# acids-ircam/RAVE

Hardware: NVIDIA H100
Metric: audio-seconds/s (v2 train step fwd+bwd, 48 kHz) (higher is better)
Workload: dtype bf16

## Files before the change

include/rave_b200.h:

```cpp
#ifndef RAVE_B200_H
#define RAVE_B200_H

#include <stddef.h>
#include <stdint.h>

#ifdef __cplusplus
extern "C" {
#endif

#define RAVE_ACT_NONE 0
#define RAVE_ACT_LEAKY 1
#define RAVE_ACT_SNAKE 2

#define RAVE_PREC_FP32 0
#define RAVE_PREC_BF16 1
#define RAVE_PREC_TF32 2

int rave_b200_version(void);
const char *rave_b200_last_error(void);
unsigned long long rave_b200_launch_count(void);

int rave_pqmf_analysis_fwd(const float *x, const float *taps, float *y, int B, int T, int Lout,
                           int ntaps, int pad_l, int flip_sign, void *stream);
int rave_pqmf_synthesis_fwd(const float *x, const float *w, float *out, int B, int L, int K,
// ... 19 lines not shown
                          int Lq, int K, int stride, int dil, int pad_l, long os_a, long os_c,
                          int act_p, int act_q, float slope, const float *alpha, void *workspace,
                          void *stream);

int rave_weight_norm_fwd(const float *v, const float *g, float *w, float *norm_out, int C0, int R,
                         void *stream);
int rave_weight_norm_bwd(const float *dw, const float *v, const float *g, const float *norm,
                         float *dv, float *dg, int C0, int R, void *stream);

int rave_act_fwd(const float *x, float *y, int B, int C, int L, int act, float slope,
                 const float *alpha, void *stream);
int rave_act_bwd(const float *dy, const float *x, float *dx, float *dalpha, int B, int C, int L,
                 int act, float slope, const float *alpha, void *stream);
int rave_am_tanh_fwd(const float *x, float *y, int B, int C, int L, void *stream);
int rave_am_tanh_bwd(const float *dy, const float *x, float *dx, int B, int C, int L, void *stream);
int rave_reparam_fwd(const float *z, const float *eps, float *zs, float *kl_sum, int B, int C, int L, void *stream);
int rave_mmd_fwd(const float *z, const float *prior, float *means, float *mmd, int B, int D, int L, void *stream);
int rave_mmd_bwd(const float *z, const float *prior, const float *g, float *dz, int B, int D, int L, void *stream);
int rave_sphere_norm_fwd(const float *z, float *out, float *norm, int B, int C, int L, void *stream);
int  rave_latent_moments(const float *z, int B, int C, int L, int D, double *state, double *work, void *stream);
long rave_latent_moments_workspace_bytes(int B, int L, int D);
int rave_sphere_norm_bwd(const float *g, const float *out, const float *norm, float *dz, int B, int C, int L,
                         void *stream);

int rave_conv1d_tc_supported(int Cin, int Cout, int K, int stride, int dil);
int rave_dilated_unit_tc_supported(int C, int L);
int rave_dilated_unit_tc_fwd(const void *xa_bf16, const void *w3t_bf16, const void *w1t_bf16, void *a1_out,
                             float *out_f32, void *out_act, int B, int C, int L, int pitch, int dil, int pad_l,
                             float slope_in, float slope_mid, int act_out, float slope_out, void *stream);
int rave_conv1d_tc_plan(int B, int Cin, int Cout, int Lout, int K);
int rave_conv1d_tc_pp_stages(int B, int Cin, int Cout, int Lout, int K, int fm, int res_bf16);
int rave_conv1d_tc_pp_fwd_stages(int B, int Cin, int Cout, int Lout, int K);
int rave_conv1d_tc_wide_stages(int B, int Cin, int Cout, int Lout, int K);
int rave_conv1d_tc_fwd(const void *xa_bf16, const void *wt_bf16, const float *bias, const float *res,
                       const void *res_bf16, const void *dact_src_bf16, const void *res_act_bf16, float res_slope,
                       float *out_f32, void *out_act_bf16,
                       int B, int Cin, int Lin, int in_pitch, int Cout, int Lout,
                       int K, int stride, int dil, int pad_l, int act, float slope, int out_rows,
                       int out_row_stride, int out_row_offset, const float *fm_d, int fm_bh, void *stream);
int rave_conv1d_tc_fwd_x3(const void *xa_bf16, const void *wt_bf16, const float *bias, const float *res,
                          const void *res_act, float res_slope, float *out_f32, void *out_act, int B, int Cin, int Lin,
                          int in_pitch, int Cout, int Lout, int K, int stride, int dil, int pad_l, int act, float slope,
                          int out_rows, int out_row_stride, int out_row_offset, int act_cs, void *stream);
int rave_conv1d_tc_wgrad_splits(int B, int Cm, int Lp, int Cn, int K);
int rave_conv1d_tc_wgrad_plan(int B, int Cm, int Lp, int Cn, int K);
int rave_time_stack_cl(const float *x, void *out_bf16, int B, int C, int T, int F, int Fp, int Cp, int kt, int pt,
                       void *stream);
int rave_time_stack_cl_bwd(const void *g_bf16, float *gx, int B, int C, int T, int F, int Fp, int Cp, int kt, int pt,
                           void *stream);
int rave_time_stack_nhwc(const float *x, void *out_bf16, int B, int C, int T, int F, long sb, long st, int Fp, int Cp, int kt,
                         int pt, void *stream);
int rave_time_stack_nhwc_bwd(const void *g_bf16, float *gx, int B, int C, int T, int F, int Fp, int Cp, int kt, int pt,
                             void *stream);
int rave_time_stack_nhwc_dil(const float *x, void *out_bf16, int B, int C, int T, int F, long sb, long st, int Fp, int Cp,
                             int kt, int pt, int dil, void *stream);
int rave_time_stack_nhwc_dil_bwd(const void *g_bf16, float *gx, int B, int C, int T, int F, int Fp, int Cp, int kt, int pt,
                                 int dil, void *stream);
int rave_l1_stats_f32(const float *t, const float *v, float *stats, long n, void *stream);
int rave_l1_grad_f32(const float *t, const float *v, const float *d, float *gt, float *gv, long n, void *stream);
int rave_leaky_fm_fwd(const float *x, float *a, float *stats, long H, float slope, void *stream);
int rave_leaky_fm_bwd(const float *a, const float *g, const float *d, float *gx, long H, float slope, void *stream);
int rave_leaky_fm_stack_fwd(const float *x, float *a, float *stats, void *xs_bf16, long Rh, int T, int F, int C, int Fp,
                            float slope, void *stream);
int rave_leaky_fm_stack_bwd(const float *a, const void *gxs_bf16, const float *ga, const float *d, float *gx, long Rh, int T,
                            int F, int C, int Fp, float slope, void *stream);
int rave_leaky_fm_stack_dil_fwd(const float *x, float *a, float *stats, void *xs_bf16, long Rh, int T, int F, int C, int Fp,
// ... 147 lines not shown
```

rave_b200/_lib.py:

```python
import ctypes
import os
from ctypes import c_float, c_int, c_long, c_longlong, c_size_t, c_ulonglong, c_void_p, c_char_p

_HERE = os.path.dirname(os.path.abspath(__file__))
LIB_PATH = os.path.join(_HERE, "csrc", "librave_b200.so")

_P, _I, _F, _L = c_void_p, c_int, c_float, c_long

SIGNATURES = {
    "rave_b200_version": (c_int, []),
    "rave_b200_last_error": (c_char_p, []),
    "rave_b200_launch_count": (c_ulonglong, []),
    "rave_pqmf_analysis_fwd": (c_int, [_P, _P, _P, _I, _I, _I, _I, _I, _I, _P]),
    "rave_pqmf_synthesis_fwd": (c_int, [_P, _P, _P, _I, _I, _I, _I, _F, _I, _P]),
    "rave_pqmf_analysis_fast": (c_int, [_P, _P, _P, _P, _I, _I, _I, _I, _I, _P]),
    "rave_pqmf_synthesis_fast": (c_int, [_P, _P, _P, _P, _I, _I, _I, _F, _I, _P]),
    "rave_conv1d_gather_f32": (c_int, [_P, _P, _P, _P, _P, _I, _I, _I, _I, _I, _I, _I, _I, _I, _L, _L,
                                       _I, _F, _P, _I, _F, _P, _P, _P]),
    "rave_conv1d_scatter_f32": (c_int, [_P, _P, _P, _P, _P, _I, _I, _I, _I, _I, _I, _I, _I, _I, _L, _L,
                                        _I, _F, _P, _I, _F, _P, _P, _P]),
    "rave_conv1d_wgrad_workspace_bytes": (c_size_t, [_I, _I, _I, _I, _I]),
    "rave_conv1d_wgrad_f32": (c_int, [_P, _P, _P, _I, _I, _I, _I, _I, _I, _I, _I, _I, _L, _L, _I, _I,
                                      _F, _P, _P, _P]),
    "rave_weight_norm_fwd": (c_int, [_P, _P, _P, _P, _I, _I, _P]),
    "rave_weight_norm_bwd": (c_int, [_P, _P, _P, _P, _P, _P, _I, _I, _P]),
    "rave_act_fwd": (c_int, [_P, _P, _I, _I, _I, _I, _F, _P, _P]),
    "rave_act_bwd": (c_int, [_P, _P, _P, _P, _I, _I, _I, _I, _F, _P, _P]),
    "rave_am_tanh_fwd": (c_int, [_P, _P, _I, _I, _I, _P]),
    "rave_am_tanh_bwd": (c_int, [_P, _P, _P, _I, _I, _I, _P]),
    "rave_reparam_fwd": (c_int, [_P, _P, _P, _P, _I, _I, _I, _P]),
    "rave_mmd_fwd": (c_int, [_P, _P, _P, _P, _I, _I, _I, _P]),
    "rave_mmd_bwd": (c_int, [_P, _P, _P, _P, _I, _I, _I, _P]),
    "rave_sphere_norm_fwd": (c_int, [_P, _P, _P, _I, _I, _I, _P]),
    "rave_sphere_norm_bwd": (c_int, [_P, _P, _P, _P, _I, _I, _I, _P]),
    "rave_latent_moments": (c_int, [_P, _I, _I, _I, _I, _P, _P, _P]),
    "rave_latent_moments_workspace_bytes": (c_long, [_I, _I, _I]),
    "rave_conv1d_tc_supported": (c_int, [_I, _I, _I, _I, _I]),
    "rave_dilated_unit_tc_supported": (c_int, [_I, _I]),
    "rave_dilated_unit_tc_fwd": (c_int, [_P, _P, _P, _P, _P, _P, _I, _I, _I, _I, _I, _I, _F, _F, _I, _F, _P]),
    "rave_conv1d_tc_plan": (c_int, [_I, _I, _I, _I, _I]),
    "rave_conv1d_tc_pp_stages": (c_int, [_I, _I, _I, _I, _I, _I, _I]),
    "rave_conv1d_tc_pp_fwd_stages": (c_int, [_I, _I, _I, _I, _I]),
    "rave_conv1d_tc_wide_stages": (c_int, [_I, _I, _I, _I, _I]),
    "rave_conv1d_tc_fwd": (c_int, [_P, _P, _P, _P, _P, _P, _P, _F, _P, _P, _I, _I, _I, _I, _I, _I, _I, _I, _I, _I, _I,
                                   _F, _I, _I, _I, _P, _I, _P]),
    "rave_conv1d_tc_fwd_x3": (c_int, [_P, _P, _P, _P, _P, _F, _P, _P, _I, _I, _I, _I, _I, _I, _I, _I, _I, _I, _I, _F, _I,
                                      _I, _I, _I, _P]),
    "rave_weight_prep_tc_multi_x3": (c_int, [_I, _P, _P]),
    "rave_ncl_to_cl_x3": (c_int, [_P, _P, _I, _I, _I, _P]),
    "rave_conv1d_tc_wgrad": (c_int, [_P, _P, _P, _P, _I, _I, _I, _I, _I, _I, _I, _I, _I, _I, _I, _P]),
    "rave_tapmajor_to_weight_f32": (c_int, [_P, _P, _I, _I, _I, _I, _I, _P]),
    "rave_conv1d_tc_wgrad_splits": (c_int, [_I, _I, _I, _I, _I]),
    "rave_conv1d_tc_wgrad_plan": (c_int, [_I, _I, _I, _I, _I]),
    "rave_time_stack_cl": (c_int, [_P, _P, _I, _I, _I, _I, _I, _I, _I, _I, _P]),
    "rave_time_stack_cl_bwd": (c_int, [_P, _P, _I, _I, _I, _I, _I, _I, _I, _I, _P]),
    "rave_time_stack_nhwc": (c_int, [_P, _P, _I, _I, _I, _I, ctypes.c_long, ctypes.c_long, _I, _I, _I, _I, _P]),
    "rave_time_stack_nhwc_bwd": (c_int, [_P, _P, _I, _I, _I, _I, _I, _I, _I, _I, _P]),
    "rave_time_stack_nhwc_dil": (c_int, [_P, _P, _I, _I, _I, _I, ctypes.c_long, ctypes.c_long, _I, _I, _I, _I, _I, _P]),
    "rave_time_stack_nhwc_dil_bwd": (c_int, [_P, _P, _I, _I, _I, _I, _I, _I, _I, _I, _I, _P]),
    "rave_l1_stats_f32": (c_int, [_P, _P, _P, ctypes.c_long, _P]),
    "rave_leaky_fm_fwd": (c_int, [_P, _P, _P, ctypes.c_long, ctypes.c_float, _P]),
    "rave_leaky_fm_bwd": (c_int, [_P, _P, _P, _P, ctypes.c_long, ctypes.c_float, _P]),
    "rave_leaky_fm_stack_fwd": (c_int, [_P, _P, _P, _P, ctypes.c_long, _I, _I, _I, _I, ctypes.c_float, _P]),
    "rave_leaky_fm_stack_bwd": (c_int, [_P, _P, _P, _P, _P, ctypes.c_long, _I, _I, _I, _I, ctypes.c_float, _P]),
    "rave_leaky_fm_stack_dil_fwd": (c_int, [_P, _P, _P, _P, ctypes.c_long, _I, _I, _I, _I, _I, ctypes.c_float, _P]),
    "rave_leaky_fm_stack_dil_bwd": (c_int, [_P, _P, _P, _P, _P, ctypes.c_long, _I, _I, _I, _I, _I, ctypes.c_float, _P]),
    "rave_l1_grad_f32": (c_int, [_P, _P, _P, _P, _P, ctypes.c_long, _P]),
    "rave_snake_cl_fwd": (c_int, [_P, _P, _P, ctypes.c_long, _I, _P]),
    "rave_snake_cl_bwd": (c_int, [_P, _P, _P, _P, _P, _P, ctypes.c_long, _I, _P]),
    "rave_adain_cl_stats": (c_int, [_P, _I, _I, _I, _I, _P, _P, _P, _P, _P, _P, _P, _P, _I, _P, _P, _P]),
    "rave_adain_snake_cl_fwd": (c_int, [_P, _P, _P, _P, _P, _I, _I, _I, _I, _P]),
    "rave_weight_prep_tc": (c_int, [_P, _P, _P, _P, _P, _I, _P, _P, _I, _I, _I, _I, _I, _I, _P]),
    "rave_weight_norm_bwd_tapmajor": (c_int, [_P, _P, _P, _P, _P, _P, _I, _I, _I, _I, _I, _I, _P]),
    "rave_conv1d_c1_fwd": (c_int, [_P, _P, _P, _P, _P, _I, _I, _I, _I, _I, _I, _I, _I, _I, _I, _F, _P]),
    "rave_conv1d_c1_wgrad_splits": (c_int, [_I, _I]),
    "rave_conv1d_c1_wgrad": (c_int, [_P, _P, _P, _I, _I, _I, _I, _I, _I, _I, _I, _I, _I, _P]),
# ... 133 lines not shown
```

rave_b200/csrc/conv_tc.cu:

```cuda
#include <string.h>

#include <type_traits>

#include "common.cuh"
#include "tc_common.cuh"

namespace rave {
namespace tc {

constexpr int BLOCK_M = 128;
constexpr int NUM_THREADS = 288;
constexpr int SMEM_MAX = 227 * 1024;

struct TcParams {
  int B, Cin, Lin, Cout, Lout, K, stride, dil, pad_l;
  int BL, BB;
  int n_lt, n_bg, n_nt;
  int num_kb;
  int act;
  float slope;
  const float *bias;
  const float *res;
  const __nv_bfloat16 *res_bf16;
  const __nv_bfloat16 *dact_src;
// ... 391 lines not shown
      const bool valid = (b < p.B) && (l < p.Lout);
      const size_t orow = (size_t)b * p.out_rows + (size_t)l * p.out_row_stride + p.out_row_offset;

      const int buf = p.nacc == 2 ? (it & 1) : 0;
      const uint32_t use = p.nacc == 2 ? (it >> 1) : it;
      if (stg) {
        if (issuer) bulk_wait_read<0>();
        named_bar_sync(1, 128);
      }
      mbar_wait(&tfull_bar[buf], use & 1);
      const uint32_t taddr = (uint32_t)(128 * buf + quad * 32) << 16;
      tc_epilogue<BLOCK_N, X3, BOXC>(p, taddr, n0, valid, orow, p.fm_d ? (b < p.fm_bh ? 1 : -1) : 0, stg, row);
      __syncwarp();
      if (lane == 0) mbar_arrive(&tempty_bar[buf]);
      if (stg) {
        fence_proxy_async();
        named_bar_sync(1, 128);
        if (issuer) {
#pragma unroll
          for (int c = 0; c < BLOCK_N; c += BOXC)
            tma_store_3d(&tmap_o, stg + (c / BOXC) * (BLOCK_M * L::OUT_SPAN), n0 + c, t.l0, t.b0);
          bulk_commit();
        }
      }
    }
    if (stg && issuer) bulk_wait_all();
  }
}

constexpr int PP_THREADS = 384;

enum PpEpi : int { PP_FM = 1, PP_RS = 2, PP_FWD = 4, PP_BIAS = 8, PP_LEAKY = 16 };

template <int BLOCK_N, int BOXC, bool FM, bool RS>
__device__ __forceinline__ void pp_epilogue(float (*d)[BLOCK_N / 2], uint8_t *slot, const TcParams &p, int w, int lane,
                                            int b0) {
  constexpr int TILE_BYTES = BLOCK_M * BLOCK_N * 2;
  uint8_t *part = slot + TILE_BYTES;
  uint8_t *skip = slot + (FM ? 2 : 1) * TILE_BYTES;
  constexpr int SPAN = BOXC * 2, JB = BOXC / 8;
  const float d0 = FM ? __ldg(p.fm_d) : 0.f, d1 = FM ? __ldg(p.fm_d + 1) : 0.f;
  const uint32_t base = stg_offset<BOXC>(16 * w + (lane >> 2), 0) + 4 * (lane & 3);
#pragma unroll
  for (int h = 0; h < 2; ++h) {
#pragma unroll
    for (int r = 0; r < 2; ++r) {
      const int row = 64 * h + 16 * w + (lane >> 2) + 8 * r;
      const float d1r = (FM && b0 + row / p.BL < p.fm_bh) ? d1 : 0.f;
#pragma unroll
      for (int j = 0; j < BLOCK_N / 8; ++j) {
        const uint32_t off = (base ^ (uint32_t)((j % JB) << 4)) + (j / JB) * (BLOCK_M * SPAN) + (64 * h + 8 * r) * SPAN;
        float v0 = d[h][4 * j + 2 * r], v1 = d[h][4 * j + 2 * r + 1];
        const uint32_t dm = *reinterpret_cast<const uint32_t *>(slot + off);
        lrelu_mask(v0, v1, dm, p.slope);
        if (FM) fm_grad(v0, v1, dm, *reinterpret_cast<const uint32_t *>(part + off), d0, d1r);
        if (RS) add_bf16_pair(v0, v1, *reinterpret_cast<const uint32_t *>(skip + off));
        __nv_bfloat162 o = __floats2bfloat162_rn(v0, v1);
        *reinterpret_cast<uint32_t *>(slot + off) = *reinterpret_cast<uint32_t *>(&o);
      }
    }
  }
}

template <int BLOCK_N, int BOXC, bool BIAS, bool LEAKY, int NH = 2>
__device__ __forceinline__ void pp_fwd_epilogue(float (*d)[BLOCK_N / 2], uint8_t *slot, const TcParams &p, int w,
                                                int lane, int n0, int h0 = 0) {
  constexpr int SPAN = BOXC * 2, JB = BOXC / 8;
  const uint32_t base = stg_offset<BOXC>(16 * w + (lane >> 2), 0) + 4 * (lane & 3);
  const uint32_t sslot = smem_u32(slot);
  const float2 *bias = reinterpret_cast<const float2 *>(p.bias + n0 + 2 * (lane & 3));
#pragma unroll
  for (int j = 0; j < BLOCK_N / 8; ++j) {
    const float2 bb = BIAS ? __ldg(bias + 4 * j) : make_float2(0.f, 0.f);
    const uint32_t col = (base ^ (uint32_t)((j % JB) << 4)) + (j / JB) * (BLOCK_M * SPAN);
#pragma unroll
    for (int h = 0; h < NH; ++h) {
#pragma unroll
      for (int r = 0; r < 2; ++r) {
        float v0 = d[h][4 * j + 2 * r], v1 = d[h][4 * j + 2 * r + 1];
        if (BIAS) {
          v0 += bb.x;
          v1 += bb.y;
        }
        if (LEAKY) {
// ... 128 lines not shown
      if (issuer) {
#pragma unroll
        for (int cb = 0; cb < BLOCK_N / BOXC; ++cb)
          tma_store_3d(tmap_o, slot + cb * BOX_BYTES, t.n0 + cb * BOXC, t.l0, t.b0);
        bulk_commit();
        bulk_wait_read<0>();
        mbar_arrive(&oempty_bar[c]);
      }
    }
    if (issuer) bulk_wait_all();
  }
}

template <int BLOCK_N, int BLOCK_K, bool FM, bool RS>
__global__ void __launch_bounds__(PP_THREADS, 1)
conv_tc_pp_kernel(const __grid_constant__ CUtensorMap tmap_a, const __grid_constant__ CUtensorMap tmap_b,
                  const __grid_constant__ CUtensorMap tmap_m, const __grid_constant__ CUtensorMap tmap_p,
                  const __grid_constant__ CUtensorMap tmap_r, const __grid_constant__ CUtensorMap tmap_o,
                  const TcParams p) {
  conv_tc_pp_body<BLOCK_N, BLOCK_K, (FM ? PP_FM : 0) | (RS ? PP_RS : 0)>(&tmap_a, &tmap_b, &tmap_m, &tmap_p, &tmap_r,
                                                                         &tmap_o, p);
}

template <int BLOCK_N, int BLOCK_K, bool BIAS, bool LEAKY>
__global__ void __launch_bounds__(PP_THREADS, 1)
conv_tc_pp_fwd_kernel(const __grid_constant__ CUtensorMap tmap_a, const __grid_constant__ CUtensorMap tmap_b,
                      const __grid_constant__ CUtensorMap tmap_o, const TcParams p) {
  conv_tc_pp_body<BLOCK_N, BLOCK_K, PP_FWD | (BIAS ? PP_BIAS : 0) | (LEAKY ? PP_LEAKY : 0)>(
      &tmap_a, &tmap_b, nullptr, nullptr, nullptr, &tmap_o, p);
}

constexpr int WIDE_N = 192;

template <int BLOCK_K, bool BIAS, bool LEAKY>
__global__ void __launch_bounds__(PP_THREADS, 1)
conv_tc_wide_kernel(const __grid_constant__ CUtensorMap tmap_a, const __grid_constant__ CUtensorMap tmap_b,
                    const __grid_constant__ CUtensorMap tmap_o, const TcParams p) {
  constexpr int BLOCK_N = WIDE_N;
  using L = SmemLayout<BLOCK_N, BLOCK_K, false>;
  constexpr int BOXC = L::OUT_BOXC;
  constexpr int BOX_BYTES = BLOCK_M * L::OUT_SPAN;
  const int STAGES = p.stages;

  extern __shared__ uint8_t smem_raw[];
  uint8_t *smem = reinterpret_cast<uint8_t *>((reinterpret_cast<uintptr_t>(smem_raw) + 1023) & ~uintptr_t(1023));
  uint64_t *full_bar = reinterpret_cast<uint64_t *>(smem + p.bar_off);
  uint64_t *empty_bar = full_bar + STAGES;
  uint64_t *oempty_bar = empty_bar + STAGES;

  const int wg = threadIdx.x >> 7;
  const int warp = threadIdx.x >> 5;
  const int lane = threadIdx.x & 31;
  const int num_tiles = p.n_lt * p.n_bg * p.n_nt;
  const int kblocks = p.K * p.num_kb;

  if (threadIdx.x == 0) {
    tma_prefetch_desc(&tmap_a);
    tma_prefetch_desc(&tmap_b);
    tma_prefetch_desc(&tmap_o);
    for (int s = 0; s < STAGES; ++s) {
      mbar_init(&full_bar[s], 1);
      mbar_init(&empty_bar[s], 8);
    }
    mbar_init(oempty_bar, 1);
    fence_barrier_init();
  }
  __syncthreads();
  griddep_launch_dependents();
  griddep_wait();

  Ring ring{full_bar, empty_bar, STAGES, 0, 0};
  if (wg == 0) {
    warpgroup_reg_dealloc<56>();
    if (warp != 0) return;
    for (int tile = blockIdx.x; tile < num_tiles; tile += gridDim.x) {
      const TileCoord t = tile_coord<BLOCK_N>(tile, p);
      for (int k = 0; k < p.K; ++k) {
        const TapOrigin o = tap_origin(k, p.dil, p.pad_l, p.stride);
        for (int kb = 0; kb < p.num_kb; ++kb)
          produce_kblock<BLOCK_N, BLOCK_K, false>(smem, ring, &tmap_a, &tmap_b, p, t, o, k, kb);
      }
    }
  } else {
    warpgroup_reg_alloc<224>();
    const int h = wg - 1;
    const int w = warp & 3;
    const bool issuer = threadIdx.x == 128;
    const uint32_t smem_base = smem_u32(smem);
    uint8_t *slot = smem + p.ops_off;
    float d[1][BLOCK_N / 2];
    int u = 0;
    for (int tile = blockIdx.x; tile < num_tiles; tile += gridDim.x, ++u) {
      const int prev = mma_mainloop<BLOCK_N, BLOCK_K, false, 1>(d, smem_base, ring, kblocks, lane, h);
      mma_drain<BLOCK_N, 1>(d, ring, prev, lane);
      const TileCoord t = tile_coord<BLOCK_N>(tile, p);
      if (issuer && u > 0) {
        bulk_wait_read<0>();
        mbar_arrive(oempty_bar);
      }
      mbar_wait(oempty_bar, (u & 1) ^ 1);
      pp_fwd_epilogue<BLOCK_N, BOXC, BIAS, LEAKY, 1>(d, slot, p, w, lane, t.n0, h);
      fence_proxy_async();
      named_bar_sync(1, 256);
      if (issuer) {
#pragma unroll
        for (int cb = 0; cb < BLOCK_N / BOXC; ++cb)
          tma_store_3d(&tmap_o, slot + cb * BOX_BYTES, t.n0 + cb * BOXC, t.l0, t.b0);
        bulk_commit();
      }
    }
    if (issuer) bulk_wait_all();
  }
}

static CUtensorMapSwizzle swizzle_enum(int bytes) {
  return bytes == 128 ? CU_TENSOR_MAP_SWIZZLE_128B : bytes == 64 ? CU_TENSOR_MAP_SWIZZLE_64B
                                                                 : CU_TENSOR_MAP_SWIZZLE_32B;
}

static int pick_block_k(int Cin) {
  if (Cin % 64 == 0) return 64;
  if (Cin % 32 == 0) return 32;
  if (Cin % 16 == 0) return 16;
  return 0;
}

static int pick_block_n(int Cout, long m_tiles) {
  const int cands[] = {128, 96, 64, 48, 32, 16};
  constexpr int NC = sizeof(cands) / sizeof(cands[0]);
  int best = 0;
  for (int c : cands) {
    if (Cout % c) continue;
    if (!best) best = c;
    if (m_tiles * (Cout / c) >= 132) return c;
  }
  for (int i = NC - 1; i >= 0; --i)
    if (Cout % cands[i] == 0 && cands[i] >= 32) return cands[i];
  return best;
}

struct TcGeometry {
  int BK, BL, BB, n_lt, n_bg, BN, n_nt, num_kb;
};
static TcGeometry tc_geometry(int B, int Cin, int Cout, int Lout) {
  TcGeometry g;
// ... 40 lines not shown
  const cuuint64_t dims[3] = {(cuuint64_t)p.Cout, (cuuint64_t)p.Lout, (cuuint64_t)p.B};
  const cuuint64_t strides[2] = {(cuuint64_t)p.Cout * 2 * p.out_row_stride, (cuuint64_t)p.Cout * 2 * p.out_rows};
  const cuuint32_t box[3] = {(cuuint32_t)L::OUT_BOXC, (cuuint32_t)p.BL, (cuuint32_t)box_b};
  const CUresult r = encode_bf16_map(m, 3, base + (size_t)p.out_row_offset * p.Cout, dims, strides, box,
                                     swizzle_enum(L::OUT_SPAN), CU_TENSOR_MAP_L2_PROMOTION_NONE);
  if (r != CUDA_SUCCESS) {
    set_error("conv1d_tc: bf16 row tensor map encode failed (%d)", (int)r);
    return 1;
  }
  return 0;
}

template <int BN, int BK, bool FWD>
constexpr bool pp_built = FWD || !(BN == 96 && BK == 64);

template <int BN, int BK, bool FWD>
constexpr int pp_stages(int nops) {
  using L = SmemLayout<BN, BK, false>;
  if (!pp_built<BN, BK, FWD>) return 0;
  const int s = (SMEM_MAX - L::FIXED - 2 * nops * BLOCK_M * BN * 2) / L::STAGE_BYTES;
  return s < 2 ? 0 : s > 8 ? 8 : s;
}

template <int BN, int BK>
static int pp_fwd_stages(int kblocks) {
  const int s = pp_stages<BN, BK, true>(1);
  TcParams q;
  plan_smem<BN, BK, false>(kblocks, q);
  return s >= q.stages && (BN == 128 || kblocks <= 24) ? s : 0;
}

static int wide_block_k(int Cin) { return pick_block_k(Cin); }
template <int BK>
constexpr int wide_ring_stages() {
  using L = SmemLayout<WIDE_N, BK, false>;
  const int s = (SMEM_MAX - L::FIXED - L::STG_BYTES) / L::STAGE_BYTES;
  return s > 8 ? 8 : s;
}
constexpr int WIDE_MIN_KBLOCKS = 12;
static int wide_stages(int Cin, int Cout, int K) {
  const int BK = wide_block_k(Cin);
  if (BK < 32 || Cout % WIDE_N || K * ceil_div(Cin, BK) < WIDE_MIN_KBLOCKS) return 0;
  return BK == 64 ? wide_ring_stages<64>() : wide_ring_stages<32>();
}

template <int BK>
static int launch_wide(const CUtensorMap &ta, const CUtensorMap &tb, TcParams p, int stages, cudaStream_t stream) {
  using L = SmemLayout<WIDE_N, BK, false>;
  p.stages = stages;
  p.ops_bytes = L::STG_BYTES;
  p.ops_off = p.stages * L::STAGE_BYTES;
  p.bar_off = p.ops_off + p.ops_bytes;
  const int grid = persistent_grid(p.n_lt * p.n_bg * p.n_nt), smem = p.bar_off + L::FIXED;
  CUtensorMap to;
  if (encode_rows_map<WIDE_N>(&to, p.out_act, p, p.BB)) return 1;
  const auto go = [&](auto bias, auto leaky) {
    return launch_tc<conv_tc_wide_kernel<BK, decltype(bias)::value, decltype(leaky)::value>>(
        "conv1d_tc", grid, PP_THREADS, smem, stream, ta, tb, to, p);
  };
  const std::true_type y;
  const std::false_type n;
  const bool leaky = p.act == RAVE_ACT_LEAKY;
  return p.bias ? (leaky ? go(y, y) : go(y, n)) : (leaky ? go(n, y) : go(n, n));
}

template <int BN, int BK, bool FWD>
static int launch_pp(const CUtensorMap &ta, const CUtensorMap &tb, TcParams p, int stages, cudaStream_t stream) {
  using L = SmemLayout<BN, BK, false>;
  p.stages = stages;
  p.ops_bytes = (1 + (p.fm_d ? 1 : 0) + (p.res_bf16 ? 1 : 0)) * BLOCK_M * BN * 2;
  p.ops_off = p.stages * L::STAGE_BYTES;
  p.bar_off = p.ops_off + 2 * p.ops_bytes;
  const int grid = persistent_grid(p.n_lt * p.n_bg * p.n_nt), smem = p.bar_off + L::FIXED;
  const std::true_type y;
  const std::false_type n;
  CUtensorMap tm, tp, tr, to;
  if (encode_rows_map<BN>(&to, p.out_act, p, p.BB)) return 1;
  if constexpr (FWD) {
    const auto go = [&](auto bias, auto leaky) {
      return launch_tc<conv_tc_pp_fwd_kernel<BN, BK, decltype(bias)::value, decltype(leaky)::value>>(
          "conv1d_tc", grid, PP_THREADS, smem, stream, ta, tb, to, p);
    };
    const bool leaky = p.act == RAVE_ACT_LEAKY;
    return p.bias ? (leaky ? go(y, y) : go(y, n)) : (leaky ? go(n, y) : go(n, n));
  } else {
    memset(&tp, 0, sizeof(tp));
    memset(&tr, 0, sizeof(tr));
    if (encode_rows_map<BN>(&tm, p.dact_src, p, p.BB)) return 1;
    if (p.fm_d && encode_rows_map<BN>(&tp, p.fm_bh > 0 ? p.dact_src : p.dact_src - p.fm_half, p, 1)) return 1;
    if (p.res_bf16 && encode_rows_map<BN>(&tr, p.res_bf16, p, p.BB)) return 1;
    const auto go = [&](auto fm, auto rs) {
      return launch_tc<conv_tc_pp_kernel<BN, BK, decltype(fm)::value, decltype(rs)::value>>(
          "conv1d_tc", grid, PP_THREADS, smem, stream, ta, tb, tm, tp, tr, to, p);
    };
    return p.fm_d ? (p.res_bf16 ? go(y, y) : go(y, n)) : (p.res_bf16 ? go(n, y) : go(n, n));
  }
// ... 39 lines not shown
  visit_tile(g.BK, g.BN, [&](auto bk, auto bn) {
    plan_smem<decltype(bn)::value, decltype(bk)::value, false>(K * g.num_kb, q);
    return 0;
  });
  return g.BN | (g.BK << 12) | (q.nacc - 1) << 24 | q.stg << 25 | q.stages << 26;
}

extern "C" int rave_conv1d_tc_pp_stages(int B, int Cin, int Cout, int Lout, int K, int fm, int res_bf16) {
  using namespace rave::tc;
  const TcGeometry g = tc_geometry(B, Cin, Cout, Lout);
  if (!g.BK || !g.BN) return 0;
  const int nops = 1 + (fm ? 1 : 0) + (res_bf16 ? 1 : 0);
  return visit_tile(g.BK, g.BN, [&](auto bk, auto bn) {
    return pp_stages<decltype(bn)::value, decltype(bk)::value, false>(nops);
  });
}

extern "C" int rave_conv1d_tc_pp_fwd_stages(int B, int Cin, int Cout, int Lout, int K) {
  using namespace rave::tc;
  const TcGeometry g = tc_geometry(B, Cin, Cout, Lout);
  if (!g.BK || !g.BN) return 0;
  return visit_tile(g.BK, g.BN, [&](auto bk, auto bn) {
    return pp_fwd_stages<decltype(bn)::value, decltype(bk)::value>(K * g.num_kb);
  });
}

extern "C" int rave_conv1d_tc_wide_stages(int B, int Cin, int Cout, int Lout, int K) {
  using namespace rave::tc;
  const TcGeometry g = tc_geometry(B, Cin, Cout, Lout);
  if (!g.BK || !g.BN) return 0;
  return wide_stages(Cin, Cout, K);
}

static int conv1d_tc_fwd_impl(const void *xa, const void *wt, const float *bias, const float *res,
                              const void *res_bf16, const void *dact_src, const void *res_act, float res_slope,
                              float *out_f32, void *out_act,
                              int B, int Cin, int Lin, int in_pitch, int Cout, int Lout,
                              int K, int stride, int dil, int pad_l, int act, float slope, int out_rows,
                              int out_row_stride, int out_row_offset, const float *fm_d, int fm_bh,
                              void *stream, int x3, int act_cs = 0) {
  using namespace rave;
  using namespace rave::tc;
  RAVE_CHECK_ARG(!x3 || (!res_bf16 && !dact_src && !fm_d),
                 "conv1d_tc(x3): the split-operand mode has no gradient epilogues (forward path only)");
  RAVE_CHECK_ARG(xa && wt && (out_f32 || out_act), "conv1d_tc: null pointer");
  RAVE_CHECK_ARG(rave_conv1d_tc_supported(Cin, Cout, K, stride, dil), "conv1d_tc: unsupported shape Cin=%d Cout=%d",
                 Cin, Cout);
  if (in_pitch <= 0) in_pitch = Lin;
  RAVE_CHECK_ARG(in_pitch >= ceil_div(Lin, stride) * stride,
                 "conv1d_tc: input pitch %d < Lin %d rounded up to the stride %d (slack rows must be zero)", in_pitch,
                 Lin, stride);
  RAVE_CHECK_ARG(act == RAVE_ACT_NONE || act == RAVE_ACT_LEAKY, "conv1d_tc: epilogue activation %d unsupported", act);
  RAVE_CHECK_ARG(act != RAVE_ACT_LEAKY || (slope >= 0.f && slope <= 1.f), "conv1d_tc: LeakyReLU slope %g outside [0, 1]",
                 (double)slope);
  RAVE_CHECK_ARG(!res_act || (res_slope > 0.f && res_slope <= 1.f), "conv1d_tc: res_slope %g outside (0, 1]",
                 (double)res_slope);
  RAVE_CHECK_ARG(((uintptr_t)bias & 15) == 0, "conv1d_tc: bias must be 16-byte aligned");
  RAVE_CHECK_ARG(((uintptr_t)xa & 15) == 0 && ((uintptr_t)wt & 15) == 0, "conv1d_tc: operands must be 16B aligned");
  RAVE_CHECK_ARG((((uintptr_t)out_f32 | (uintptr_t)out_act | (uintptr_t)res | (uintptr_t)res_bf16 | (uintptr_t)dact_src |
                   (uintptr_t)res_act) & 31) == 0,
                 "conv1d_tc: epilogue tensors must be 32-byte aligned (256-bit row segments)");
  RAVE_CHECK_ARG(get_encode_fn(), "conv1d_tc: cuTensorMapEncodeTiled not available");

  const TcGeometry g = tc_geometry(B, Cin, Cout, Lout);
  RAVE_CHECK_ARG(g.BN > 0, "conv1d_tc: no BLOCK_N for Cout=%d", Cout);
  const bool bf16_only = out_act && !res && !res_act && !out_f32;
  const bool pp_dgrad = bf16_only && dact_src && !bias && act == RAVE_ACT_NONE;
  const bool pp_fwd = bf16_only && !dact_src && !res_bf16 && !fm_d;
  const int wide = !x3 && pp_fwd ? wide_stages(Cin, Cout, K) : 0;
  const int BK = wide ? wide_block_k(Cin) : g.BK, BN = wide ? WIDE_N : g.BN;
  const CUtensorMapL2promotion promo = BK == 64 ? CU_TENSOR_MAP_L2_PROMOTION_L2_256B : CU_TENSOR_MAP_L2_PROMOTION_NONE;
  TcParams p;
  p.B = B; p.Cin = Cin; p.Lin = Lin; p.Cout = Cout; p.Lout = Lout; p.K = K; p.stride = stride; p.dil = dil;
  p.pad_l = pad_l; p.act = act; p.slope = slope; p.bias = bias; p.res = res; p.out_f32 = out_f32;
  p.res_bf16 = (const __nv_bfloat16 *)res_bf16; p.dact_src = (const __nv_bfloat16 *)dact_src;
  p.res_act = (const __nv_bfloat16 *)res_act;
  p.res_inv_slope = (res_act && res_slope > 0.f) ? 1.f / res_slope : 1.f;
  p.out_act = (__nv_bfloat16 *)out_act;
  p.out_rows = out_rows > 0 ? out_rows : Lout;
  p.out_row_stride = out_row_stride > 0 ? out_row_stride : 1;
  p.out_row_offset = out_row_offset;
  RAVE_CHECK_ARG(!fm_d || (dact_src && slope > 0.f && ((fm_bh > 0 && 2 * fm_bh == B) || (fm_bh < 0 && -fm_bh == B))),
                 "conv1d_tc: the fused feature-matching gradient needs dact_src and a [real; fake] batch (B=%d, fm_bh=%d)",
                 B, fm_bh);
  p.fm_d = fm_d;
  p.fm_bh = fm_bh > 0 ? fm_bh : 0;
  p.fm_half = (long)(fm_bh > 0 ? fm_bh : -fm_bh) * p.out_rows * Cout;
  p.act_ld = x3 ? 2 * Cout : Cout;
  p.act_cs = act_cs > 0 ? act_cs : Cout;
  RAVE_CHECK_ARG(!x3 || (Cout % p.act_cs == 0 && p.act_cs % 16 == 0),
                 "conv1d_tc(x3): %d channels per position do not tile the %d-column rows in 16-column chunks", p.act_cs,
                 Cout);
  RAVE_CHECK_ARG(!x3 || !res_act || p.act_cs == Cout, "conv1d_tc(x3): res_act needs one position per row");
  p.BL = g.BL; p.BB = g.BB; p.n_lt = g.n_lt; p.n_bg = g.n_bg;
  p.n_nt = Cout / BN;
  p.num_kb = ceil_div(Cin, BK);

  CUtensorMap ta, tb;
  {
    const cuuint64_t ca = (cuuint64_t)Cin * (x3 ? 2 : 1);
    const cuuint64_t dims[4] = {ca, (cuuint64_t)stride, (cuuint64_t)ceil_div(Lin, stride), (cuuint64_t)B};
    const cuuint64_t strides[3] = {ca * 2, ca * 2 * stride, ca * 2 * in_pitch};
// ... 367 lines not shown
```

Measured before the change: 2480.

## Route bf16 data-gradient convolutions through the wide 192-column persistent kernel

Extends the wide BLOCK_N=192 persistent TMA/wgmma kernel to the backward data-gradient path. It adds TMA loads of the activation-mask operand (and the paired feature-matching operand) issued by the producer warp, a dedicated store warp, and extra barriers that hand the epilogue tile off between the math and store warps. The aim is to reuse the wider N tile for dgrad so each A tile is loaded fewer times and the mainloop runs more efficiently. In exchange the extra operand buffers take shared memory and leave fewer ring stages, and small-K shapes are gated out by minimum-kblock thresholds.

```diff
diff --git a/include/rave_b200.h b/include/rave_b200.h
--- a/include/rave_b200.h
+++ b/include/rave_b200.h
@@ -75,6 +75,7 @@
 int rave_conv1d_tc_pp_stages(int B, int Cin, int Cout, int Lout, int K, int fm, int res_bf16);
 int rave_conv1d_tc_pp_fwd_stages(int B, int Cin, int Cout, int Lout, int K);
 int rave_conv1d_tc_wide_stages(int B, int Cin, int Cout, int Lout, int K);
+int rave_conv1d_tc_wide_dgrad_stages(int B, int Cin, int Cout, int Lout, int K, int fm);
 int rave_conv1d_tc_fwd(const void *xa_bf16, const void *wt_bf16, const float *bias, const float *res,
                        const void *res_bf16, const void *dact_src_bf16, const void *res_act_bf16, float res_slope,
                        float *out_f32, void *out_act_bf16,
diff --git a/rave_b200/_lib.py b/rave_b200/_lib.py
--- a/rave_b200/_lib.py
+++ b/rave_b200/_lib.py
@@ -42,6 +42,7 @@
     "rave_conv1d_tc_pp_stages": (c_int, [_I, _I, _I, _I, _I, _I, _I]),
     "rave_conv1d_tc_pp_fwd_stages": (c_int, [_I, _I, _I, _I, _I]),
     "rave_conv1d_tc_wide_stages": (c_int, [_I, _I, _I, _I, _I]),
+    "rave_conv1d_tc_wide_dgrad_stages": (c_int, [_I, _I, _I, _I, _I, _I]),
     "rave_conv1d_tc_fwd": (c_int, [_P, _P, _P, _P, _P, _P, _P, _F, _P, _P, _I, _I, _I, _I, _I, _I, _I, _I, _I, _I, _I,
                                    _F, _I, _I, _I, _P, _I, _P]),
     "rave_conv1d_tc_fwd_x3": (c_int, [_P, _P, _P, _P, _P, _F, _P, _P, _I, _I, _I, _I, _I, _I, _I, _I, _I, _I, _I, _F, _I,
diff --git a/rave_b200/csrc/conv_tc.cu b/rave_b200/csrc/conv_tc.cu
--- a/rave_b200/csrc/conv_tc.cu
+++ b/rave_b200/csrc/conv_tc.cu
@@ -447,9 +447,9 @@
 
 enum PpEpi : int { PP_FM = 1, PP_RS = 2, PP_FWD = 4, PP_BIAS = 8, PP_LEAKY = 16 };
 
-template <int BLOCK_N, int BOXC, bool FM, bool RS>
+template <int BLOCK_N, int BOXC, bool FM, bool RS, int NH = 2>
 __device__ __forceinline__ void pp_epilogue(float (*d)[BLOCK_N / 2], uint8_t *slot, const TcParams &p, int w, int lane,
-                                            int b0) {
+                                            int b0, int h0 = 0) {
   constexpr int TILE_BYTES = BLOCK_M * BLOCK_N * 2;
   uint8_t *part = slot + TILE_BYTES;
   uint8_t *skip = slot + (FM ? 2 : 1) * TILE_BYTES;
@@ -457,14 +457,15 @@
   const float d0 = FM ? __ldg(p.fm_d) : 0.f, d1 = FM ? __ldg(p.fm_d + 1) : 0.f;
   const uint32_t base = stg_offset<BOXC>(16 * w + (lane >> 2), 0) + 4 * (lane & 3);
 #pragma unroll
-  for (int h = 0; h < 2; ++h) {
+  for (int h = 0; h < NH; ++h) {
 #pragma unroll
     for (int r = 0; r < 2; ++r) {
-      const int row = 64 * h + 16 * w + (lane >> 2) + 8 * r;
+      const int row = 64 * (h0 + h) + 16 * w + (lane >> 2) + 8 * r;
       const float d1r = (FM && b0 + row / p.BL < p.fm_bh) ? d1 : 0.f;
 #pragma unroll
       for (int j = 0; j < BLOCK_N / 8; ++j) {
-        const uint32_t off = (base ^ (uint32_t)((j % JB) << 4)) + (j / JB) * (BLOCK_M * SPAN) + (64 * h + 8 * r) * SPAN;
+        const uint32_t off =
+            (base ^ (uint32_t)((j % JB) << 4)) + (j / JB) * (BLOCK_M * SPAN) + (64 * (h0 + h) + 8 * r) * SPAN;
         float v0 = d[h][4 * j + 2 * r], v1 = d[h][4 * j + 2 * r + 1];
         const uint32_t dm = *reinterpret_cast<const uint32_t *>(slot + off);
         lrelu_mask(v0, v1, dm, p.slope);
@@ -659,14 +660,17 @@
 
 constexpr int WIDE_N = 192;
 
-template <int BLOCK_K, bool BIAS, bool LEAKY>
-__global__ void __launch_bounds__(PP_THREADS, 1)
-conv_tc_wide_kernel(const __grid_constant__ CUtensorMap tmap_a, const __grid_constant__ CUtensorMap tmap_b,
-                    const __grid_constant__ CUtensorMap tmap_o, const TcParams p) {
+template <int BLOCK_K, int E>
+__device__ __forceinline__ void conv_tc_wide_body(const CUtensorMap *tmap_a, const CUtensorMap *tmap_b,
+                                                  const CUtensorMap *tmap_m, const CUtensorMap *tmap_p,
+                                                  const CUtensorMap *tmap_o, const TcParams &p) {
   constexpr int BLOCK_N = WIDE_N;
   using L = SmemLayout<BLOCK_N, BLOCK_K, false>;
   constexpr int BOXC = L::OUT_BOXC;
   constexpr int BOX_BYTES = BLOCK_M * L::OUT_SPAN;
+  constexpr bool FWD = E & PP_FWD, FM = E & PP_FM;
+  static_assert(!(E & PP_RS), "the wide kernel has no gradient-skip operand set");
+  static_assert(!FWD || !FM, "the forward epilogue has no gradient operands");
   const int STAGES = p.stages;
 
   extern __shared__ uint8_t smem_raw[];
@@ -674,6 +678,9 @@
   uint64_t *full_bar = reinterpret_cast<uint64_t *>(smem + p.bar_off);
   uint64_t *empty_bar = full_bar + STAGES;
   uint64_t *oempty_bar = empty_bar + STAGES;
+  uint64_t *swritten_bar = oempty_bar + 1;
+  uint64_t *ofull_bar = oempty_bar + 2;
+  uint8_t *slot = smem + p.ops_off;
 
   const int wg = threadIdx.x >> 7;
   const int warp = threadIdx.x >> 5;
@@ -682,14 +689,20 @@
   const int kblocks = p.K * p.num_kb;
 
   if (threadIdx.x == 0) {
-    tma_prefetch_desc(&tmap_a);
-    tma_prefetch_desc(&tmap_b);
-    tma_prefetch_desc(&tmap_o);
+    tma_prefetch_desc(tmap_a);
+    tma_prefetch_desc(tmap_b);
+    tma_prefetch_desc(tmap_o);
+    if constexpr (!FWD) tma_prefetch_desc(tmap_m);
+    if constexpr (FM) tma_prefetch_desc(tmap_p);
     for (int s = 0; s < STAGES; ++s) {
       mbar_init(&full_bar[s], 1);
       mbar_init(&empty_bar[s], 8);
     }
     mbar_init(oempty_bar, 1);
+    if constexpr (!FWD) {
+      mbar_init(swritten_bar, 8);
+      mbar_init(ofull_bar, 1);
+    }
     fence_barrier_init();
   }
   __syncthreads();
@@ -699,45 +712,106 @@
   Ring ring{full_bar, empty_bar, STAGES, 0, 0};
   if (wg == 0) {
     warpgroup_reg_dealloc<56>();
-    if (warp != 0) return;
-    for (int tile = blockIdx.x; tile < num_tiles; tile += gridDim.x) {
-      const TileCoord t = tile_coord<BLOCK_N>(tile, p);
-      for (int k = 0; k < p.K; ++k) {
-        const TapOrigin o = tap_origin(k, p.dil, p.pad_l, p.stride);
-        for (int kb = 0; kb < p.num_kb; ++kb)
-          produce_kblock<BLOCK_N, BLOCK_K, false>(smem, ring, &tmap_a, &tmap_b, p, t, o, k, kb);
-      }
+    if (warp == 0) {
+      const int ops_kb = (STAGES < kblocks ? STAGES : kblocks) - 1;
+      int u = 0;
+      for (int tile = blockIdx.x; tile < num_tiles; tile += gridDim.x, ++u) {
+        const TileCoord t = tile_coord<BLOCK_N>(tile, p);
+        for (int k = 0; k < p.K; ++k) {
+          const TapOrigin o = tap_origin(k, p.dil, p.pad_l, p.stride);
+          for (int kb = 0; kb < p.num_kb; ++kb) {
+            produce_kblock<BLOCK_N, BLOCK_K, false>(smem, ring, tmap_a, tmap_b, p, t, o, k, kb);
+            if (!FWD && k * p.num_kb + kb == ops_kb) {
+              mbar_wait(oempty_bar, (u & 1) ^ 1);
+              if (elect_one()) {
+                mbar_arrive_expect_tx(ofull_bar, p.ops_bytes);
+                for (int cb = 0; cb < BLOCK_N / BOXC; ++cb) {
+                  tma_load_3d(slot + cb * BOX_BYTES, tmap_m, ofull_bar, t.n0 + cb * BOXC, t.l0, t.b0);
+                  if (FM) {
+                    for (int i = 0; i < p.BB; ++i) {
+                      const int b = t.b0 + i;
+                      const int pb = p.fm_bh > 0 ? (b < p.fm_bh ? b + p.fm_bh : b - p.fm_bh) : b;
+                      tma_load_3d(slot + BLOCK_M * BLOCK_N * 2 + cb * BOX_BYTES + i * p.BL * L::OUT_SPAN, tmap_p,
+                                  ofull_bar, t.n0 + cb * BOXC, t.l0, pb);
+                    }
+                  }
+                }
+              }
+              __syncwarp();
+            }
+          }
+        }
+      }
+    } else if (!FWD && warp == 1) {
+      int u = 0;
+      for (int tile = blockIdx.x; tile < num_tiles; tile += gridDim.x, ++u) {
+        const TileCoord t = tile_coord<BLOCK_N>(tile, p);
+        mbar_wait(swritten_bar, u & 1);
+        if (lane == 0) {
+#pragma unroll
+          for (int cb = 0; cb < BLOCK_N / BOXC; ++cb)
+            tma_store_3d(tmap_o, slot + cb * BOX_BYTES, t.n0 + cb * BOXC, t.l0, t.b0);
+          bulk_commit();
+          bulk_wait_read<0>();
+          mbar_arrive(oempty_bar);
+        }
+        __syncwarp();
+      }
+      if (lane == 0) bulk_wait_all();
     }
   } else {
     warpgroup_reg_alloc<224>();
     const int h = wg - 1;
     const int w = warp & 3;
-    const bool issuer = threadIdx.x == 128;
+    const bool issuer = FWD && threadIdx.x == 128;
     const uint32_t smem_base = smem_u32(smem);
-    uint8_t *slot = smem + p.ops_off;
     float d[1][BLOCK_N / 2];
     int u = 0;
     for (int tile = blockIdx.x; tile < num_tiles; tile += gridDim.x, ++u) {
       const int prev = mma_mainloop<BLOCK_N, BLOCK_K, false, 1>(d, smem_base, ring, kblocks, lane, h);
       mma_drain<BLOCK_N, 1>(d, ring, prev, lane);
       const TileCoord t = tile_coord<BLOCK_N>(tile, p);
-      if (issuer && u > 0) {
-        bulk_wait_read<0>();
-        mbar_arrive(oempty_bar);
-      }
-      mbar_wait(oempty_bar, (u & 1) ^ 1);
-      pp_fwd_epilogue<BLOCK_N, BOXC, BIAS, LEAKY, 1>(d, slot, p, w, lane, t.n0, h);
-      fence_proxy_async();
-      named_bar_sync(1, 256);
-      if (issuer) {
-#pragma unroll
-        for (int cb = 0; cb < BLOCK_N / BOXC; ++cb)
-          tma_store_3d(&tmap_o, slot + cb * BOX_BYTES, t.n0 + cb * BOXC, t.l0, t.b0);
-        bulk_commit();
+      if constexpr (FWD) {
+        if (issuer && u > 0) {
+          bulk_wait_read<0>();
+          mbar_arrive(oempty_bar);
+        }
+        mbar_wait(oempty_bar, (u & 1) ^ 1);
+        pp_fwd_epilogue<BLOCK_N, BOXC, (E & PP_BIAS) != 0, (E & PP_LEAKY) != 0, 1>(d, slot, p, w, lane, t.n0, h);
+        fence_proxy_async();
+        named_bar_sync(1, 256);
+        if (issuer) {
+#pragma unroll
+          for (int cb = 0; cb < BLOCK_N / BOXC; ++cb)
+            tma_store_3d(tmap_o, slot + cb * BOX_BYTES, t.n0 + cb * BOXC, t.l0, t.b0);
+          bulk_commit();
+        }
+      } else {
+        mbar_wait(ofull_bar, u & 1);
+        pp_epilogue<BLOCK_N, BOXC, FM, false, 1>(d, slot, p, w, lane, t.b0, h);
+        fence_proxy_async();
+        __syncwarp();
+        if (lane == 0) mbar_arrive(swritten_bar);
       }
     }
     if (issuer) bulk_wait_all();
   }
+}
+
+template <int BLOCK_K, bool BIAS, bool LEAKY>
+__global__ void __launch_bounds__(PP_THREADS, 1)
+conv_tc_wide_kernel(const __grid_constant__ CUtensorMap tmap_a, const __grid_constant__ CUtensorMap tmap_b,
+                    const __grid_constant__ CUtensorMap tmap_o, const TcParams p) {
+  conv_tc_wide_body<BLOCK_K, PP_FWD | (BIAS ? PP_BIAS : 0) | (LEAKY ? PP_LEAKY : 0)>(&tmap_a, &tmap_b, nullptr,
+                                                                                     nullptr, &tmap_o, p);
+}
+
+template <int BLOCK_K, bool FM>
+__global__ void __launch_bounds__(PP_THREADS, 1)
+conv_tc_wide_dgrad_kernel(const __grid_constant__ CUtensorMap tmap_a, const __grid_constant__ CUtensorMap tmap_b,
+                          const __grid_constant__ CUtensorMap tmap_m, const __grid_constant__ CUtensorMap tmap_p,
+                          const __grid_constant__ CUtensorMap tmap_o, const TcParams p) {
+  conv_tc_wide_body<BLOCK_K, FM ? PP_FM : 0>(&tmap_a, &tmap_b, &tmap_m, &tmap_p, &tmap_o, p);
 }
 
 static CUtensorMapSwizzle swizzle_enum(int bytes) {
@@ -844,36 +918,54 @@
 
 static int wide_block_k(int Cin) { return pick_block_k(Cin); }
 template <int BK>
-constexpr int wide_ring_stages() {
+constexpr int wide_ring_stages(int nops) {
   using L = SmemLayout<WIDE_N, BK, false>;
-  const int s = (SMEM_MAX - L::FIXED - L::STG_BYTES) / L::STAGE_BYTES;
+  const int s = (SMEM_MAX - L::FIXED - nops * L::STG_BYTES) / L::STAGE_BYTES;
   return s > 8 ? 8 : s;
 }
 constexpr int WIDE_MIN_KBLOCKS = 12;
 static int wide_stages(int Cin, int Cout, int K) {
   const int BK = wide_block_k(Cin);
   if (BK < 32 || Cout % WIDE_N || K * ceil_div(Cin, BK) < WIDE_MIN_KBLOCKS) return 0;
-  return BK == 64 ? wide_ring_stages<64>() : wide_ring_stages<32>();
+  return BK == 64 ? wide_ring_stages<64>(1) : wide_ring_stages<32>(1);
+}
+constexpr int WIDE_DGRAD_MIN_KBLOCKS = 6, WIDE_DGRAD_FM_MIN_KBLOCKS = 24;
+static int wide_dgrad_stages(int Cin, int Cout, int K, bool fm, bool res_bf16) {
+  const int BK = wide_block_k(Cin);
+  if (res_bf16 || BK < 32 || Cout % WIDE_N) return 0;
+  if (K * ceil_div(Cin, BK) < (fm ? WIDE_DGRAD_FM_MIN_KBLOCKS : WIDE_DGRAD_MIN_KBLOCKS)) return 0;
+  const int nops = fm ? 2 : 1;
+  return BK == 64 ? wide_ring_stages<64>(nops) : wide_ring_stages<32>(nops);
 }
 
 template <int BK>
 static int launch_wide(const CUtensorMap &ta, const CUtensorMap &tb, TcParams p, int stages, cudaStream_t stream) {
   using L = SmemLayout<WIDE_N, BK, false>;
   p.stages = stages;
-  p.ops_bytes = L::STG_BYTES;
+  p.ops_bytes = (p.dact_src && p.fm_d ? 2 : 1) * L::STG_BYTES;
   p.ops_off = p.stages * L::STAGE_BYTES;
   p.bar_off = p.ops_off + p.ops_bytes;
   const int grid = persistent_grid(p.n_lt * p.n_bg * p.n_nt), smem = p.bar_off + L::FIXED;
-  CUtensorMap to;
-  if (encode_rows_map<WIDE_N>(&to, p.out_act, p, p.BB)) return 1;
-  const auto go = [&](auto bias, auto leaky) {
-    return launch_tc<conv_tc_wide_kernel<BK, decltype(bias)::value, decltype(leaky)::value>>(
-        "conv1d_tc", grid, PP_THREADS, smem, stream, ta, tb, to, p);
-  };
   const std::true_type y;
   const std::false_type n;
-  const bool leaky = p.act == RAVE_ACT_LEAKY;
-  return p.bias ? (leaky ? go(y, y) : go(y, n)) : (leaky ? go(n, y) : go(n, n));
+  CUtensorMap tm, tp, to;
+  if (encode_rows_map<WIDE_N>(&to, p.out_act, p, p.BB)) return 1;
+  if (!p.dact_src) {
+    const auto go = [&](auto bias, auto leaky) {
+      return launch_tc<conv_tc_wide_kernel<BK, decltype(bias)::value, decltype(leaky)::value>>(
+          "conv1d_tc", grid, PP_THREADS, smem, stream, ta, tb, to, p);
+    };
+    const bool leaky = p.act == RAVE_ACT_LEAKY;
+    return p.bias ? (leaky ? go(y, y) : go(y, n)) : (leaky ? go(n, y) : go(n, n));
+  }
+  memset(&tp, 0, sizeof(tp));
+  if (encode_rows_map<WIDE_N>(&tm, p.dact_src, p, p.BB)) return 1;
+  if (p.fm_d && encode_rows_map<WIDE_N>(&tp, p.fm_bh > 0 ? p.dact_src : p.dact_src - p.fm_half, p, 1)) return 1;
+  const auto go = [&](auto fm) {
+    return launch_tc<conv_tc_wide_dgrad_kernel<BK, decltype(fm)::value>>("conv1d_tc", grid, PP_THREADS, smem, stream,
+                                                                          ta, tb, tm, tp, to, p);
+  };
+  return p.fm_d ? go(y) : go(n);
 }
 
 template <int BN, int BK, bool FWD>
@@ -979,6 +1071,13 @@
   return wide_stages(Cin, Cout, K);
 }
 
+extern "C" int rave_conv1d_tc_wide_dgrad_stages(int B, int Cin, int Cout, int Lout, int K, int fm) {
+  using namespace rave::tc;
+  const TcGeometry g = tc_geometry(B, Cin, Cout, Lout);
+  if (!g.BK || !g.BN) return 0;
+  return wide_dgrad_stages(Cin, Cout, K, fm != 0, false);
+}
+
 static int conv1d_tc_fwd_impl(const void *xa, const void *wt, const float *bias, const float *res,
                               const void *res_bf16, const void *dact_src, const void *res_act, float res_slope,
                               float *out_f32, void *out_act,
@@ -1014,7 +1113,8 @@
   const bool bf16_only = out_act && !res && !res_act && !out_f32;
   const bool pp_dgrad = bf16_only && dact_src && !bias && act == RAVE_ACT_NONE;
   const bool pp_fwd = bf16_only && !dact_src && !res_bf16 && !fm_d;
-  const int wide = !x3 && pp_fwd ? wide_stages(Cin, Cout, K) : 0;
+  const int wide = x3 ? 0 : pp_fwd ? wide_stages(Cin, Cout, K)
+                         : pp_dgrad ? wide_dgrad_stages(Cin, Cout, K, fm_d != nullptr, res_bf16 != nullptr) : 0;
   const int BK = wide ? wide_block_k(Cin) : g.BK, BN = wide ? WIDE_N : g.BN;
   const CUtensorMapL2promotion promo = BK == 64 ? CU_TENSOR_MAP_L2_PROMOTION_L2_256B : CU_TENSOR_MAP_L2_PROMOTION_NONE;
   TcParams p;
```

Result: no change. 2502 (median of 6 runs) (+0.9%).
